# JohnsonLabJanelia/laserCalib

Hardware: NVIDIA B200
Metric: LM_iters_per_sec (higher is better)
Workload: dtype f64

## Files before the change

include/lcba.h:

```cpp
#ifndef LCBA_H
#define LCBA_H

#include <stddef.h>
#include <stdint.h>

#ifdef __cplusplus
extern "C" {
#endif

#define LCBA_VERSION 100
#define LCBA_CAM_PARAMS 11
#define LCBA_MAX_CAMERAS 64
#define LCBA_MAX_TRACE 512

enum {
  LCBA_OK = 0,
  LCBA_E_ARG = -1,
  LCBA_E_CUDA = -2,
  LCBA_E_STATE = -3,
  LCBA_E_UNSUPPORTED = -4,
  LCBA_E_NONFINITE = -5,
  LCBA_E_NCCL = -6
};

// ... 81 lines not shown

int lcba_residuals(lcba_t* h, const double* x_or_null, double* r_out, double* cost_out);

int lcba_jacobian_blocks(lcba_t* h, const double* x_or_null, double* Jc, double* Jp);

int lcba_sparsity_indices(lcba_t* h, int32_t C, int64_t P, int64_t N, const int64_t* cam_idx,
                          const int64_t* pt_idx, int32_t* indices_out);

int lcba_solve(lcba_t* h, const lcba_options* opt, lcba_result* res);
int lcba_get_trace(lcba_t* h, lcba_trace_row* rows, int32_t max_rows);
typedef void (*lcba_iteration_cb)(const lcba_trace_row* row, void* user);
int lcba_set_iteration_callback(lcba_t* h, lcba_iteration_cb cb, void* user);
int lcba_get_grad(lcba_t* h, double* g_out );
int lcba_get_profile(lcba_t* h, lcba_kernel_stat* stats, int32_t max_stats, int32_t* n_out);

int lcba_linearize(lcba_t* h, double lam, double* S_out, double* rhs_out, double* grad_out,
                   double* scale_inv_out, double* cost_out);

int lcba_time_device(lcba_t* h, int32_t what, int32_t reps, double* ms_out);

int lcba_nccl_unique_id(void* id_out128);
int lcba_comm_init(lcba_t* h, int32_t rank, int32_t nranks, const void* id128);

int lcba_debug_tr2d(double B00, double B01, double B11, double g0, double g1, double Delta,
                    double* p_out2, int* newton_out);

int lcba_debug_chol(lcba_t* h, int32_t n, const double* A, const double* rhs, double mu, const double* d,
                    int32_t grid, double* x_out, double* factor_out, int32_t* fail_out);

#define LCBA_STEP_SCALARS 18
int lcba_debug_step(lcba_t* h, double lam, double mu, int32_t mode, double* pc_out, double* pp_out,
                    double* scalars_out);

int lcba_debug_schur_stats(lcba_t* h, long long* out, int max_ctas, int* nkinds, int* nslices);

int lcba_debug_mma_plan(int32_t C, int32_t sm_count, int32_t* units_out, int32_t max_kinds,
                        int32_t* nslices_out, int32_t* ok_out);

int lcba_debug_i8_plan(int32_t C, int64_t P, int32_t sm_count, int32_t* tiles_out, int32_t max_tiles,
                       int32_t* work_out, int32_t max_work, int32_t* nwork_out, int32_t* nrg_out,
                       int64_t* nkb_out);

int lcba_debug_i8_cover_plan(int32_t C, int64_t P, int32_t sm_count, int32_t which, int32_t* tiles_out,
                             int32_t max_tiles, int32_t* work_out, int32_t max_work, int32_t* nwork_out,
                             int32_t* nrg_out, int64_t* nkb_out, int32_t* cover_out, double* model_out);

int lcba_debug_i8_fallback(lcba_t* h);

int lcba_debug_peer_reduce(lcba_t* h, int enable);

int lcba_host_is_nondecreasing_i64(const int64_t* v, int64_t n, int32_t threads);

#ifdef __cplusplus
}
#endif
#endif
```

lasercalib_b200/_cabi.py:

```python
from __future__ import annotations

import ctypes as C
import os

import numpy as np

_PKG = os.path.dirname(os.path.abspath(__file__))
LIB_PATH = os.path.join(_PKG, "liblcba.so")

LCBA_MAX_TRACE = 512
E_NAMES = {-1: "LCBA_E_ARG", -2: "LCBA_E_CUDA", -3: "LCBA_E_STATE", -4: "LCBA_E_UNSUPPORTED",
           -5: "LCBA_E_NONFINITE", -6: "LCBA_E_NCCL"}

SYMBOLS = ["lcba_version", "lcba_create", "lcba_destroy", "lcba_last_error", "lcba_default_options",
           "lcba_set_problem", "lcba_set_problem_shard", "lcba_set_params", "lcba_get_params", "lcba_rotate", "lcba_project",
           "lcba_unproject", "lcba_residuals", "lcba_jacobian_blocks", "lcba_sparsity_indices", "lcba_solve",
           "lcba_get_trace", "lcba_get_grad", "lcba_get_profile", "lcba_linearize",
           "lcba_time_device", "lcba_nccl_unique_id", "lcba_comm_init", "lcba_debug_tr2d",
           "lcba_sq_normal", "lcba_debug_schur_stats", "lcba_debug_mma_plan",
           "lcba_set_iteration_callback", "lcba_debug_i8_plan", "lcba_host_is_nondecreasing_i64", "lcba_debug_peer_reduce",
           "lcba_debug_i8_fallback", "lcba_debug_chol", "lcba_debug_step", "lcba_debug_i8_cover_plan"]

STEP_SCALARS = ["reg_term", "Delta", "Jg2", "aa", "ab", "bb", "JAA", "JAB", "JBB", "gtgt", "gtp", "pp",
                "c0", "c1", "predicted", "step_h_norm", "step_norm", "chol_fail"]


class Options(C.Structure):
    _fields_ = [("ftol", C.c_double), ("xtol", C.c_double), ("gtol", C.c_double),
                ("max_nfev", C.c_int64), ("verbose", C.c_int32), ("profile", C.c_int32),
                ("max_iterations", C.c_int32), ("fix_cameras", C.c_int32), ("shared_intrinsics", C.c_int32), ("reserved", C.c_int32 * 3)]


class TraceRow(C.Structure):
    _fields_ = [("iteration", C.c_int64), ("nfev", C.c_int64), ("cost", C.c_double),
                ("cost_reduction", C.c_double), ("step_norm", C.c_double),
                ("optimality", C.c_double), ("delta", C.c_double), ("reg_term", C.c_double)]


class Result(C.Structure):
    _fields_ = [("cost", C.c_double), ("optimality", C.c_double), ("initial_cost", C.c_double),
                ("nfev", C.c_int64), ("njev", C.c_int64), ("iterations", C.c_int64),
                ("status", C.c_int32), ("n_trace", C.c_int32), ("solve_ms", C.c_double),
                ("gpu_launches", C.c_int64), ("reserved", C.c_double * 6)]


class KernelStat(C.Structure):
    _fields_ = [("name", C.c_char * 32), ("launches", C.c_int64), ("total_ms", C.c_double)]


ITERATION_CB = C.CFUNCTYPE(None, C.POINTER(TraceRow), C.c_void_p)


def _row_dict(r):
    return dict(iteration=r.iteration, nfev=r.nfev, cost=r.cost, cost_reduction=r.cost_reduction,
# ... 29 lines not shown
    lib.lcba_default_options.argtypes = [C.POINTER(Options)]
    lib.lcba_default_options.restype = None
    lib.lcba_set_problem.argtypes = [vp, i32, i64, i64, vp, vp, vp, vp, vp, vp]
    lib.lcba_set_problem_shard.argtypes = [vp, i32, i64, i64, vp, vp, vp, vp, vp, vp, i64]
    lib.lcba_set_params.argtypes = [vp, vp, vp]
    lib.lcba_get_params.argtypes = [vp, vp, vp]
    lib.lcba_rotate.argtypes = [vp, i64, vp, vp, vp]
    lib.lcba_project.argtypes = [vp, i64, vp, vp, vp]
    lib.lcba_unproject.argtypes = [vp, i64, vp, vp, i64, vp, vp, vp, vp, vp]
    lib.lcba_residuals.argtypes = [vp, vp, vp, pd]
    lib.lcba_jacobian_blocks.argtypes = [vp, vp, vp, vp]
    lib.lcba_sparsity_indices.argtypes = [vp, i32, i64, i64, vp, vp, vp]
    lib.lcba_solve.argtypes = [vp, C.POINTER(Options), C.POINTER(Result)]
    lib.lcba_get_trace.argtypes = [vp, C.POINTER(TraceRow), i32]
    lib.lcba_set_iteration_callback.argtypes = [vp, ITERATION_CB, vp]
    lib.lcba_get_grad.argtypes = [vp, vp]
    lib.lcba_get_profile.argtypes = [vp, C.POINTER(KernelStat), i32, C.POINTER(i32)]
    lib.lcba_linearize.argtypes = [vp, dbl, vp, vp, vp, vp, pd]
    lib.lcba_time_device.argtypes = [vp, i32, i32, pd]
    lib.lcba_nccl_unique_id.argtypes = [vp]
    lib.lcba_comm_init.argtypes = [vp, i32, i32, vp]
    lib.lcba_sq_normal.argtypes = [vp, i32, vp, pd, vp, vp]
    lib.lcba_debug_mma_plan.argtypes = [i32, i32, vp, i32, C.POINTER(i32), C.POINTER(i32)]
    lib.lcba_debug_schur_stats.argtypes = [vp, vp, C.c_int, C.POINTER(C.c_int), C.POINTER(C.c_int)]
    lib.lcba_debug_i8_plan.argtypes = [i32, i64, i32, vp, i32, vp, i32, C.POINTER(i32), C.POINTER(i32), C.POINTER(i64)]
    lib.lcba_debug_i8_cover_plan.argtypes = [i32, i64, i32, i32, vp, i32, vp, i32, C.POINTER(i32), C.POINTER(i32),
                                             C.POINTER(i64), C.POINTER(i32), vp]
    lib.lcba_host_is_nondecreasing_i64.argtypes = [vp, i64, i32]
    lib.lcba_debug_peer_reduce.argtypes = [vp, i32]
    lib.lcba_debug_i8_fallback.argtypes = [vp]
    lib.lcba_debug_tr2d.argtypes = [dbl, dbl, dbl, dbl, dbl, dbl, pd, C.POINTER(C.c_int)]
    lib.lcba_debug_chol.argtypes = [vp, i32, vp, vp, dbl, vp, i32, vp, vp, C.POINTER(i32)]
    lib.lcba_debug_step.argtypes = [vp, dbl, dbl, i32, vp, vp, vp]
    _lib = lib
    return lib


def _ptr(a):
    return None if a is None else a.ctypes.data_as(C.c_void_p)


def _f64(a, shape=None):
    a = np.ascontiguousarray(a, dtype=np.float64)
    if shape is not None:
        a = a.reshape(shape)
    return a


def _i64(a):
    return np.ascontiguousarray(a, dtype=np.int64)


class Engine:

    def __init__(self, device=-1):
        self.lib = load()
        h = C.c_void_p()
        rc = self.lib.lcba_create(C.byref(h), int(device))
        if rc != 0:
            raise LcbaError(rc, self.lib.lcba_last_error(None).decode())
        self.h = h
        self.C = self.P = self.N = 0
        self.generation = 0

    def close(self):
        if getattr(self, "h", None):
            self.lib.lcba_destroy(self.h)
            self.h = None
# ... 176 lines not shown
                                          _ptr(work), work.shape[0], C.byref(nwork), C.byref(nrg), C.byref(nkb),
                                          C.byref(cover), _ptr(model))
        if nt < 0:
            raise LcbaError(nt, "lcba_debug_i8_cover_plan: bad arguments")
        return dict(tiles=tiles[:nt].copy(), work=work[:nwork.value].copy(), nrg=nrg.value, nkb=nkb.value,
                    cover=bool(cover.value), executed_ops=model[0], cycles=model[1], strip_cycles=model[2],
                    cover_cycles=model[3])

    def debug_chol(self, A, rhs, mu=0.0, d=None, grid=0):
        A = _f64(A)
        n = A.shape[0]
        if A.shape != (n, n):
            raise ValueError("A must be square")
        rhs = _f64(rhs).ravel()
        d = None if d is None else _f64(d).ravel()
        if rhs.size != n or (d is not None and d.size != n):
            raise ValueError("rhs and d must have n entries")
        x = np.empty(n)
        factor = np.empty((n + 1, n))
        fail = C.c_int32()
        self._check(self.lib.lcba_debug_chol(self.h, n, _ptr(A), _ptr(rhs), float(mu), _ptr(d), int(grid),
                                             _ptr(x), _ptr(factor), C.byref(fail)))
        return x, factor, fail.value

    STEP_FULL, STEP_FIX_CAMERAS, STEP_SHARED_INTRINSICS = 0, 1, 2

    def debug_step(self, lam, mu=0.0, mode=0):
        pc = np.empty(11 * self.C)
        pp = np.empty(3 * self.P)
        sc = np.empty(len(STEP_SCALARS))
        self._check(self.lib.lcba_debug_step(self.h, float(lam), float(mu), int(mode), _ptr(pc), _ptr(pp), _ptr(sc)))
        return pc, pp, dict(zip(STEP_SCALARS, sc.tolist()))

    def time_device(self, what, reps=10):
        ms = C.c_double()
        self._check(self.lib.lcba_time_device(self.h, int(what), int(reps), C.byref(ms)))
        return ms.value

    @staticmethod
    def nccl_unique_id():
        lib = load()
        buf = C.create_string_buffer(128)
        rc = lib.lcba_nccl_unique_id(buf)
        if rc != 0:
            raise LcbaError(rc, lib.lcba_last_error(None).decode())
        return buf.raw

    def comm_init(self, rank, nranks, unique_id=None):
        buf = None if unique_id is None else C.create_string_buffer(bytes(unique_id), 128)
        self._check(self.lib.lcba_comm_init(self.h, int(rank), int(nranks), buf))


def debug_tr2d(B00, B01, B11, g0, g1, Delta):
    lib = load()
    p = (C.c_double * 2)()
    newton = C.c_int()
    lib.lcba_debug_tr2d(B00, B01, B11, g0, g1, Delta, p, C.byref(newton))
    return np.array([p[0], p[1]]), bool(newton.value)
```

lasercalib_b200/csrc/lcba.cu:

```cuda
#include <dlfcn.h>
#include <math.h>
#include <stdio.h>
#include <string.h>
#include <algorithm>
#include <map>
#include <string>
#include <thread>
#include <vector>

#include <nvtx3/nvToolsExt.h>

#include "common.cuh"
#include "control.cuh"
#include "dense.cuh"
#include "eval.cuh"
#include "ingest.cuh"
#include "linearize.cuh"
#include "dense_passes.cuh"
#include "schur.cuh"
#include "schur_mma.cuh"
#include "schur_i8.cuh"
#include "peer_reduce.cuh"
#include "variants.cuh"

// ... 63 lines not shown
  double *d_S = nullptr, *d_Lf = nullptr, *d_rhs = nullptr, *d_Sred = nullptr, *d_Spart = nullptr;
  int* d_fail = nullptr;
  long long* d_stats = nullptr;
  Ctl* d_ctl = nullptr;
  Ctl* h_ctl = nullptr;
  int lin_grid = 0, obs_grid = 0, pt_grid = 0;
  SchurPlan plan;
  SchurKind* d_kinds = nullptr;
  SchurHw* d_hws = nullptr;
  MmaPlan mplan;
  MmaKind* d_mkinds = nullptr;
  double *d_U = nullptr, *d_Upart = nullptr;
  int camn_grid = 0, camn_pb = 0;
  bool use_mma = false;
  bool use_dense = false;
  bool use_pt = false;
  int pt_mode = 1;
  int ptp_grid = 0;
  int dp_pb = 0, dp_grid_lin = 0, dp_grid = 0;
  double *d_dpart = nullptr, *d_dred = nullptr;
  double* d_Yg = nullptr;
  bool use_i8 = false;
  bool i8_tma = false;
  I8Maps i8maps;
  I8Plan i8plan;
  I8Work* d_i8work = nullptr;
  I8Tile* d_i8tiles = nullptr;
  unsigned char* d_i8planes = nullptr;
  double *d_i8partial = nullptr, *d_i8rmax = nullptr;
  int* d_i8erow = nullptr;
  int* d_i8gate = nullptr;
  double* d_i8mrow = nullptr;
  bool i8_guard = true;
  int i8_gx_max = 0, i8_gx_make = 0, i8_groups = 0;
  double2* d_rout = nullptr;
  double *d_Jc = nullptr, *d_Jp = nullptr;
  uint32_t* d_pair_start = nullptr;
  double* d_pair_w = nullptr;
  long long n_pairs = 0;
  struct GraphSlot { cudaGraphExec_t exec = nullptr; long long launches = 0; int key = -1; };
  GraphSlot g_body[2], g_lin[2];
  bool use_graphs = true;
  int solves_on_problem = 0;
  long long graph_replays = 0;
  lcba_iteration_cb iter_cb = nullptr;
  void* iter_cb_user = nullptr;
  std::vector<lcba_trace_row> trace;
  bool prof_on = false;
  cudaEvent_t ev0 = nullptr, ev1 = nullptr;
  std::map<std::string, std::pair<long long, double>> prof;
  long long launches = 0;
  ncclComm_t comm = nullptr;
  int rank = 0, nranks = 1;
  int fix_cameras = 0, shared_intr = 0;
  double *d_pred = nullptr, *d_scl_red = nullptr;
  double *d_sqpart = nullptr, *d_sqout = nullptr, *d_theta = nullptr;
  int sq_grid = 0, sq_K = 0;
};

static std::string g_last_error;
static ncclComm_t g_comm = nullptr;
static int g_comm_rank = -1, g_comm_nranks = 0, g_comm_device = -1;
struct PeerState {
  bool ok = false;
  void* block = nullptr;
  void* opened[PEER_MAX_RANKS] = {};
  PeerPtrs ptrs = {};
// ... 122 lines not shown
    return LCBA_E_CUDA;
  }
  cudaDeviceProp prop;
  cudaGetDeviceProperties(&prop, device);
  h->sm_count = prop.multiProcessorCount;
  h->smem_optin = prop.sharedMemPerBlockOptin;
  cudaStreamCreateWithFlags(&h->stream, cudaStreamNonBlocking);
  {
    cudaMemPool_t pool;
    if (cudaDeviceGetDefaultMemPool(&pool, device) == cudaSuccess) {
      unsigned long long keep = ~0ull;
      cudaMemPoolSetAttribute(pool, cudaMemPoolAttrReleaseThreshold, &keep);
    }
  }
  cudaEventCreate(&h->ev0);
  cudaEventCreate(&h->ev1);
  cudaMallocHost((void**)&h->h_ctl, sizeof(Ctl));
  {
    const void* big_smem_kernels[] = {(const void*)k_linearize, (const void*)k_backsub,
                                      (const void*)k_schur<true, 160>, (const void*)k_schur<false, 160>,
                                      (const void*)k_schur<true, 128>, (const void*)k_schur<false, 128>,
                                      (const void*)k_residual, (const void*)k_cam_normal, (const void*)k_make_Y,
                                      (const void*)k_schur_mma<1, false>, (const void*)k_schur_mma<2, false>,
                                      (const void*)k_schur_mma<3, false>, (const void*)k_schur_mma<4, false>,
                                      (const void*)k_schur_mma<5, false>, (const void*)k_schur_mma<6, false>,
                                      (const void*)k_schur_mma<1, true>, (const void*)k_schur_mma<2, true>,
                                      (const void*)k_schur_mma<3, true>, (const void*)k_schur_mma<4, true>,
                                      (const void*)k_schur_mma<5, true>, (const void*)k_schur_mma<6, true>,
                                      (const void*)k_sq_camonly<true>, (const void*)k_sq_camonly<false>,
                                      (const void*)k_linearize_dense, (const void*)k_residual_dense,
                                      (const void*)k_jdot_dense, (const void*)k_backsub_dense,
                                      (const void*)k_residual_pt, (const void*)k_jdot_pt, (const void*)k_backsub_pt,
                                      (const void*)k_i8_syrk<true>, (const void*)k_i8_syrk<false>, (const void*)k_i8_make,
                                      (const void*)k_jdot,      (const void*)k_jacobian_blocks};
    for (const void* f : big_smem_kernels) {
      cudaFuncAttributes fa;
      e = cudaFuncGetAttributes(&fa, f);
      if (e == cudaSuccess)
        e = cudaFuncSetAttribute(f, cudaFuncAttributeMaxDynamicSharedMemorySize,
                                 (int)(h->smem_optin - fa.sharedSizeBytes));
      if (e != cudaSuccess) {
        set_error(nullptr, std::string("lcba_create: shared-memory opt-in: ") + cudaGetErrorString(e));
        delete h;
        return LCBA_E_CUDA;
      }
    }
  }
  *out = h;
  return LCBA_OK;
}

extern "C" void lcba_destroy(lcba_t* h) {
  if (!h) return;
  cudaSetDevice(h->device);
  h->comm = nullptr;
  dev_free_all(h);
  if (h->stream) cudaStreamSynchronize(h->stream);
  if (h->h_ctl) cudaFreeHost(h->h_ctl);
  if (h->ev0) cudaEventDestroy(h->ev0);
  if (h->ev1) cudaEventDestroy(h->ev1);
  if (h->stream) cudaStreamDestroy(h->stream);
  delete h;
}

static inline unsigned nblk(long long n, int t) { return (unsigned)std::max<long long>(1, (n + t - 1) / t); }

// ... 184 lines not shown
  LCBA_TRY(dev_alloc(h, &h->d_campart, (size_t)h->lin_grid * C * CAMSUM));
  LCBA_TRY(dev_alloc(h, &h->d_part, (size_t)max_grid * 16));
  h->plan = make_schur_plan(C, h->sm_count, h->smem_optin - 2048);
  LCBA_TRY(dev_alloc(h, &h->d_kinds, h->plan.kinds.size()));
  LCBA_TRY(dev_alloc(h, &h->d_hws, h->plan.hws.size()));
  LCBA_CUDA(h, cudaMemcpyAsync(h->d_kinds, h->plan.kinds.data(), h->plan.kinds.size() * sizeof(SchurKind),
                               cudaMemcpyHostToDevice, st));
  LCBA_CUDA(h, cudaMemcpyAsync(h->d_hws, h->plan.hws.data(), h->plan.hws.size() * sizeof(SchurHw),
                               cudaMemcpyHostToDevice, st));
  LCBA_TRY(dev_alloc(h, &h->d_Sred, h->plan.part_stride));
  h->use_mma = false;
  h->d_mkinds = nullptr; h->d_U = nullptr; h->d_Upart = nullptr; h->d_Yg = nullptr;
  int max_slices = h->plan.nslices;
  {
    const char* de = getenv("LCBA_MMA_DENSITY");
    const double min_density = de ? atof(de) : 0.25;
    const bool dense = (double)h->n_pairs >= min_density * (double)P * C;
    const char* env = getenv("LCBA_SCHUR_MMA");
    const bool want = env ? atoi(env) != 0 : (dense && C >= 8);
    if (want && C <= MMA_MAX_CAMERAS) {
      {
        const char* ie = getenv("LCBA_SCHUR_I8");
        h->use_i8 = ie ? atoi(ie) != 0 : P >= 32768;
      }
      if (h->use_i8) {
        {
          const char* pe = getenv("LCBA_I8_PLAN");
          const int which = !pe ? 0 : (strcmp(pe, "strip") == 0 ? 1 : (strcmp(pe, "cover") == 0 ? 2 : 0));
          h->i8plan = make_i8_best_plan(C, P, h->sm_count, which);
        }
        const I8Plan& ip = h->i8plan;
        h->i8_groups = (C + I8_GROUP_CAMS - 1) / I8_GROUP_CAMS;
        h->i8_gx_max = (int)std::max<long long>(1, std::min<long long>(ip.nkb, (long long)h->sm_count * 4 / h->i8_groups));
        h->i8_gx_make = (int)std::max<long long>(1, std::min<long long>(ip.nkb, (long long)h->sm_count * 3 / h->i8_groups));
        LCBA_TRY(dev_alloc(h, &h->d_i8work, ip.work.size()));
        LCBA_TRY(dev_alloc(h, &h->d_i8tiles, ip.tiles.size()));
        LCBA_CUDA(h, cudaMemcpyAsync(h->d_i8work, ip.work.data(), ip.work.size() * sizeof(I8Work), cudaMemcpyHostToDevice, st));
        LCBA_CUDA(h, cudaMemcpyAsync(h->d_i8tiles, ip.tiles.data(), ip.tiles.size() * sizeof(I8Tile), cudaMemcpyHostToDevice, st));
        LCBA_TRY(dev_alloc(h, &h->d_i8planes, ip.plane_bytes));
        {
          const char* te = getenv("LCBA_I8_TMA");
          h->i8_tma = !(te && atoi(te) == 0) && i8_encode_maps(ip, h->d_i8planes, &h->i8maps);
          if (!h->i8_tma) memset(&h->i8maps, 0, sizeof(h->i8maps));
        }
        LCBA_TRY(dev_alloc(h, &h->d_i8partial, ip.work.size() * 128 * 64));
        LCBA_TRY(dev_alloc(h, &h->d_i8rmax, (size_t)h->i8_gx_max * ip.NRG * 8));
        LCBA_TRY(dev_alloc(h, &h->d_i8erow, (size_t)ip.NRG * 8));
        LCBA_TRY(dev_alloc(h, &h->d_i8gate, 1));
        LCBA_TRY(dev_alloc(h, &h->d_i8mrow, (size_t)ip.NRG * 8));
        LCBA_CUDA(h, cudaMemsetAsync(h->d_i8gate, 0, sizeof(int), st));
        {
          const char* ge = getenv("LCBA_I8_GUARD");
          h->i8_guard = !(ge && atoi(ge) == 0);
        }
      }
      bool pre = false;
      if (!h->use_i8) {
        int rp = C * 12 + 2;
        while (rp % 16 != 4) ++rp;
        const size_t need = (size_t)(P + 1) * 3 * rp * 8;
        size_t fr = 0, tot = 0;
        const char* pe = getenv("LCBA_MMA_PRE");
        pre = cudaMemGetInfo(&fr, &tot) == cudaSuccess && need < fr / 3 && !(pe && atoi(pe) == 0);
        if (pre) LCBA_TRY(dev_alloc(h, &h->d_Yg, need / 8));
      }
      h->mplan = make_mma_plan(C, h->sm_count, h->smem_optin - 2048, !pre);
      LCBA_TRY(dev_alloc(h, &h->d_mkinds, h->mplan.kinds.size()));
// ... 273 lines not shown
        h->d_Vg, h->d_pts[w], h->d_scl_p, h->d_gt_p, h->P, first, h->d_part));
  KL(h, "reduce", k_reduce_scalars<<<PP_K, 256, 0, h->stream>>>(h->d_part, h->pt_grid, PP_K, pp, 3));
  LCBA_TRY(allreduce(h, h->d_camsum, (size_t)C * CAMSUM + 1 + 3, NCCL_SUM));
  LCBA_TRY(allreduce(h, pp + 3, 1, NCCL_MAX));
  KL(h, "ctl", k_ctl_lin<<<1, 256, 0, h->stream>>>(h->d_camsum, h->d_cams[w], h->d_scl_c, h->d_gt_c,
                                                   h->d_g_c, C, h->d_ctl, first, h->fix_cameras, h->shared_intr));
  KL(h, "ctl", k_ctl_lin2<<<1, 1, 0, h->stream>>>(pp, h->d_ctl, first));
  return check_launch(h, "linearize pass");
}

static int pass_jdot(lcba_t* h) {
  NvtxRange nvtx_("lcba:jdot");
  const int C = h->C, w = h->cur;
  const size_t smem = ((size_t)C * CAMTAB + (size_t)C * NCP) * 8;
  if (h->use_pt) {
    KL(h, "jdot", k_jdot_pt<<<h->ptp_grid, PT_THREADS, smem, h->stream>>>(
          h->d_tab[w], h->d_pts[w], h->d_w, h->d_obs_start, h->d_mask, h->d_gt_c, h->d_gt_p, h->P, C, h->d_part));
    KL(h, "reduce", k_reduce_scalars<<<1, 256, 0, h->stream>>>(h->d_part, h->ptp_grid, 1, h->d_red, 1));
  } else if (h->use_dense && h->pt_mode == 2) {
    KL(h, "jdot", k_jdot_dense<<<h->dp_grid, DP_THREADS, (size_t)C * CAMTAB * 8, h->stream>>>(
          h->d_tab[w], h->d_pts[w], h->d_w, h->d_obs_start, h->d_mask, h->d_gt_c, h->d_gt_p, h->P, C,
          h->dp_pb, h->d_part));
    KL(h, "reduce", k_reduce_scalars<<<1, 256, 0, h->stream>>>(h->d_part, h->dp_grid, 1, h->d_red, 1));
  } else {
  KL(h, "jdot", k_jdot<<<h->obs_grid, 256, smem, h->stream>>>(
        h->d_tab[w], h->d_pts[w], h->d_cam, h->d_pt, h->d_w, h->d_gt_c, h->d_gt_p, h->N, C, h->d_part));
  KL(h, "reduce", k_reduce_scalars<<<1, 256, 0, h->stream>>>(h->d_part, h->obs_grid, 1, h->d_red, 1));
  }
  LCBA_TRY(allreduce(h, h->d_red, 1, NCCL_SUM));
  KL(h, "ctl", k_ctl_reg<<<1, 1, 0, h->stream>>>(h->d_red, h->d_ctl));
  return check_launch(h, "jdot pass");
}

static int pass_schur(lcba_t* h, const double* lam_host_or_null) {
  NvtxRange nvtx_("lcba:schur");
  const int C = h->C, w = h->cur, n = C * NCP;
  const SchurPlan& pl = h->plan;
  const double lam_arg = lam_host_or_null ? *lam_host_or_null : 0.0;
  const Ctl* ctl_arg = lam_host_or_null ? nullptr : h->d_ctl;
  KL(h, "point_factor", k_point_factor<<<nblk(h->P, 256), 256, 0, h->stream>>>(
        h->d_Vg, h->d_scl_p, lam_arg, ctl_arg, h->P, h->d_Lz));
  if (h->use_mma) {
    const MmaPlan& mp = h->mplan;
    if (!h->use_dense) {
    const size_t smem_u = ((size_t)((C * CAMTAB + 1) & ~1) + (size_t)h->camn_pb * C) * 8;
    KL(h, "cam_normal", k_cam_normal<<<h->camn_grid, 256, smem_u, h->stream>>>(
          h->d_tab[w], h->d_pts[w], h->d_pair_w, h->d_pair_start, h->d_mask, h->P, C, h->camn_pb, h->d_Upart));
    KL(h, "reduce", k_reduce_cols<<<nblk(C * CAMN_VALS, RC_COLS), RC_COLS * RC_ROWS, 0, h->stream>>>(
          h->d_Upart, h->camn_grid, C * CAMN_VALS, h->d_U));
    }
    const int nt = (NCP * C + 1 + 7) / 8, last = nt - 6 * ((nt + 5) / 6 - 1);
    if (h->use_i8) {
      const I8Plan& ip = h->i8plan;
      const int RP = ip.NRG * 8;
      const size_t smem_rm = ((size_t)I8_GROUP_CAMS * CAMTAB + 192) * 4;
      KL(h, "i8_rowmax", k_i8_rowmax<<<dim3(h->i8_gx_max, h->i8_groups), 192, smem_rm, h->stream>>>(
            h->d_tab[w], h->d_pts[w], h->d_pair_w, h->d_pair_start, h->d_mask, h->d_Lz, h->P, C, RP, h->d_i8rmax));
      KL(h, "i8_rowmax", k_i8_rowexp<<<nblk(RP, 128), 128, 0, h->stream>>>(h->d_i8rmax, h->i8_gx_max, NCP * C + 1, RP,
                                                                     h->d_i8erow, h->d_i8mrow));
      KL(h, "make_Y", k_i8_make<<<dim3(h->i8_gx_make, h->i8_groups), 192, i8_make_smem_bytes(), h->stream>>>(
            h->d_tab[w], h->d_pts[w], h->d_pair_w, h->d_pair_start, h->d_mask, h->d_Lz, h->P, C, ip.NRG, h->d_i8erow,
            h->d_i8planes));
      if (h->i8_tma)
        KL(h, "schur", k_i8_syrk<true><<<(unsigned)ip.work.size(), I8_THREADS, ip.smem_bytes, h->stream>>>(
              h->i8maps, h->d_i8planes, ip.NRG, h->d_i8work, h->d_i8partial, h->d_fail, h->d_stats));
      else
        KL(h, "schur", k_i8_syrk<false><<<(unsigned)ip.work.size(), I8_THREADS, ip.smem_bytes, h->stream>>>(
              h->i8maps, h->d_i8planes, ip.NRG, h->d_i8work, h->d_i8partial, h->d_fail, h->d_stats));
      KL(h, "schur_reduce", k_i8_gather<<<dim3((unsigned)ip.tiles.size(), 16), 256, 0, h->stream>>>(
            h->d_i8partial, h->d_i8tiles, C, ip.cover ? 1 : 0, h->d_i8erow, pl.npairs, h->d_Sred));
      KL(h, "schur_reduce", k_add_cam_blocks<<<nblk(C * 121, 128), 128, 0, h->stream>>>(h->d_U, C, h->d_Sred));
      if (h->i8_guard) {
        KL(h, "i8_check", k_i8_check<<<1, 256, 0, h->stream>>>(h->d_i8mrow, C, h->d_Sred, h->d_i8gate));
#define LCBA_MMA_GATED(L)                                                                            \
  KL(h, "i8_fallback", (k_schur_mma<L, false><<<dim3(mp.nslices, mp.nkinds), MMA_THREADS, mp.smem_bytes, h->stream>>>( \
          nullptr, h->d_tab[w], h->d_pts[w], h->d_pair_w, h->d_pair_start, h->d_mask, h->d_Lz, h->P, h->n_pairs, C, \
          h->d_mkinds, mp.nslices, pl.part_stride, pl.npairs, h->d_Spart, nullptr, h->d_i8gate)))
        switch (last) {
          case 1: LCBA_MMA_GATED(1); break;
          case 2: LCBA_MMA_GATED(2); break;
          case 3: LCBA_MMA_GATED(3); break;
          case 4: LCBA_MMA_GATED(4); break;
          case 5: LCBA_MMA_GATED(5); break;
          default: LCBA_MMA_GATED(6); break;
        }
#undef LCBA_MMA_GATED
        KL(h, "i8_fallback", k_i8_fallback_finish<<<h->sm_count, 256, 0, h->stream>>>(
              h->d_i8gate, h->d_Spart, mp.nslices, pl.part_stride, h->d_U, C, h->d_Sred));
      }
    } else {
    if (h->d_Yg) {
      const int pbk = MAKEY_THREADS / C, rpk = mp.kinds[0].rp;
      const size_t smem_y = ((size_t)((C * CAMTAB + 1) & ~1) + (size_t)3 * pbk * rpk) * 8;
      const int grid_y = (int)std::min<long long>((h->P + pbk - 1) / pbk, (long long)h->sm_count * 5);
      KL(h, "make_Y", k_make_Y<<<grid_y, MAKEY_THREADS, smem_y, h->stream>>>(
// ... 832 lines not shown
  if (mode < 0 || mode > 2) { set_error(h, "lcba_debug_step: mode must be 0, 1 or 2"); return LCBA_E_ARG; }
  cudaSetDevice(h->device);
  Ctl init;
  memset(&init, 0, sizeof(init));
  init.term = -1;
  LCBA_CUDA(h, cudaMemcpyAsync(h->d_ctl, &init, sizeof(Ctl), cudaMemcpyHostToDevice, h->stream));
  h->fix_cameras = mode == 1 ? 1 : 0;
  h->shared_intr = mode == 2 ? 1 : 0;
  LCBA_TRY(pass_linearize(h, 1));
  LCBA_TRY(pass_jdot(h));
  if (h->fix_cameras) {
    KL(h, "point_factor", k_point_factor<<<nblk(h->P, 256), 256, 0, h->stream>>>(
          h->d_Vg, h->d_scl_p, lam, nullptr, h->P, h->d_Lz));
    LCBA_CUDA(h, cudaMemsetAsync(h->d_pc, 0, (size_t)h->C * NCP * 8, h->stream));
    LCBA_CUDA(h, cudaMemsetAsync(h->d_fail, 0, 2 * sizeof(int), h->stream));
  } else {
    LCBA_TRY(pass_schur(h, &lam));
    LCBA_TRY(pass_camera_solve(h, mu));
  }
  LCBA_TRY(pass_backsub(h));
  if (pc_out) LCBA_CUDA(h, cudaMemcpyAsync(pc_out, h->d_pc, (size_t)h->C * NCP * 8, cudaMemcpyDeviceToHost, h->stream));
  if (pp_out) LCBA_CUDA(h, cudaMemcpyAsync(pp_out, h->d_gn_p, (size_t)h->P * 3 * 8, cudaMemcpyDeviceToHost, h->stream));
  LCBA_TRY(read_ctl(h));
  if (scalars_out) {
    const Ctl& c = *h->h_ctl;
    const double v[LCBA_STEP_SCALARS] = {c.reg_term, c.Delta, c.Jg2, c.aa, c.ab, c.bb, c.JAA, c.JAB, c.JBB,
                                         c.gtgt, c.gtp, c.pp, c.c0, c.c1, c.predicted, c.step_h_norm,
                                         c.step_norm, (double)c.chol_fail};
    memcpy(scalars_out, v, sizeof(v));
  }
  return LCBA_OK;
}

extern "C" int lcba_host_is_nondecreasing_i64(const int64_t* v, int64_t n, int32_t threads) {
  if (!v || n < 2) return 1;
  const int nt = (int)std::max<int64_t>(1, std::min<int64_t>(std::min<int64_t>(threads, 16), n / (1 << 20)));
  std::vector<int> ok(nt, 1);
  auto piece = [&](int i) {
    const int64_t a = n * i / nt, b = std::min<int64_t>(n, n * (i + 1) / nt + 1);
    int64_t bad = 0;
    for (int64_t k = a + 1; k < b; ++k) bad |= (int64_t)(v[k] < v[k - 1]);
    ok[i] = bad ? 0 : 1;
  };
  if (nt == 1) { piece(0); return ok[0]; }
  std::vector<std::thread> th;
  int started = 1;
  try {
    for (int i = 1; i < nt; ++i) { th.emplace_back(piece, i); started = i + 1; }
  } catch (...) {
  }
  piece(0);
  for (int i = started; i < nt; ++i) piece(i);
  for (auto& t : th) t.join();
  for (int i = 0; i < nt; ++i) if (!ok[i]) return 0;
  return 1;
}
```

lasercalib_b200/csrc/schur_i8.cuh:

```cuda
#pragma once
#include <cuda.h>
#include <algorithm>
#include <vector>
#include "common.cuh"
#include "schur_mma.cuh"

namespace lcba {

constexpr int I8_NS = 6;
constexpr int I8_DMAX = 6;
constexpr int I8_ND = I8_DMAX + 1;
constexpr int I8_PTS = 21;
constexpr int I8_STAGES = 3;
constexpr int I8_FLUSH = 224;
constexpr int I8_THREADS = 192;
constexpr int I8_RG_BYTES = 512;
constexpr int I8_GROUP_CAMS = 8;
constexpr int I8_GROUP_RG = 13;
constexpr int I8_GROUP_ROWS = I8_GROUP_RG * 8;

struct I8Work {
  int m_rg0, m_nrg, m2_rg0, m2_nrg, n_rg0, n_nrg, n2_rg0, n2_nrg;
  int kb0, kb1;
  int map_a, map_b1, map_b2, pad;
// ... 363 lines not shown
      for (int qq = 0; qq < I8_PTS; ++qq) m = fmaxf(m, s_red[qq * gc + t]);
      out[(c0 + t) * NCP + a] = (double)m;
    }
  }
  if (g == gridDim.y - 1) {
    __syncthreads();
    s_red[t] = zthread ? mz : 0.0f;
    __syncthreads();
    if (t == 0) {
      float m = 0.0f;
      for (int i = 168; i < 168 + I8_PTS; ++i) m = fmaxf(m, s_red[i]);
      out[NCP * C] = (double)m;
    }
  }
}

__global__ void k_i8_rowexp(const double* __restrict__ rmax_part, int nb, int R, int RP, int* __restrict__ e_row,
                            double* __restrict__ m_row) {
  const int r = blockIdx.x * blockDim.x + threadIdx.x;
  if (r >= RP) return;
  double m = 0.0;
  if (r < R) for (int b = 0; b < nb; ++b) m = fmax(m, rmax_part[(size_t)b * RP + r]);
  int e = 0;
  if (m > 0.0 && m < 1e300) { frexp(m * 1.001, &e); e += 2; }
  e_row[r] = e;
  m_row[r] = m;
}

__device__ __forceinline__ unsigned long long i8_encode(double v, double scale) {
  const long long T = __double2ll_rn(v * scale);
  return (unsigned long long)(T + 0x808080808080LL) ^ 0x808080808080ULL;
}

constexpr int I8_VAL_LD = 65;
inline size_t i8_make_smem_bytes() {
  return (size_t)I8_GROUP_CAMS * CAMTAB * 8 + (size_t)I8_GROUP_ROWS * 8 + (size_t)I8_GROUP_ROWS * I8_VAL_LD * 8;
}

__global__ void __launch_bounds__(192, 3)
k_i8_make(const double* __restrict__ tab, const double* __restrict__ pts, const double* __restrict__ wgt,
          const uint32_t* __restrict__ obs_start, const unsigned long long* __restrict__ mask,
          const double* __restrict__ Lz, long long P, int C, int NRG, const int* __restrict__ e_row,
          unsigned char* __restrict__ planes) {
  extern __shared__ __align__(16) unsigned char s_raw[];
  double* s_tab = reinterpret_cast<double*>(s_raw);
  double* s_scale = s_tab + I8_GROUP_CAMS * CAMTAB;
  unsigned long long* s_val = reinterpret_cast<unsigned long long*>(s_scale + I8_GROUP_ROWS);
  const int t = threadIdx.x, g = blockIdx.y, lane = t & 31, wid = t >> 5;
  const int c0 = g * I8_GROUP_CAMS, gc = min(I8_GROUP_CAMS, C - c0);
  const int rg0 = 11 * g;
  const int nrgl = (g == (int)gridDim.y - 1) ? NRG - rg0 : 11;
  for (int i = t; i < gc * CAMTAB; i += blockDim.x) s_tab[i] = tab[c0 * CAMTAB + i];
  for (int i = t; i < I8_GROUP_ROWS; i += blockDim.x)
    s_scale[i] = (rg0 * 8 + i < NRG * 8) ? ldexp(1.0, 8 * I8_NS - e_row[rg0 * 8 + i]) : 0.0;
  for (int i = t; i < I8_GROUP_ROWS * I8_VAL_LD; i += blockDim.x) s_val[i] = 0ull;
  __syncthreads();
  const bool worker = t < I8_PTS * gc;
  const int slot = worker ? t / gc : 0;
  const int q = slot < 16 ? (slot >> 1) + 8 * (slot & 1) : slot, cl = worker ? t % gc : 0, cam = c0 + cl;
  const bool zthread = (g == (int)gridDim.y - 1) && t >= 168 && t < 168 + I8_PTS;
  const int zrow = NCP * C - rg0 * 8;
  const long long nkb = (P + I8_PTS - 1) / I8_PTS;
  unsigned long long n_m = 0ull;
  double n_X[3] = {0, 0, 0}, n_li[6] = {0, 0, 0, 0, 0, 0};
  auto prefetch = [&](long long kb) {
    n_m = 0ull;
    const long long p = kb * I8_PTS + q;
    if (worker && kb < nkb && p < P) {
      n_m = mask[p];
#pragma unroll
      for (int a = 0; a < 3; ++a) n_X[a] = pts[3 * p + a];
#pragma unroll
      for (int a = 0; a < 6; ++a) n_li[a] = Lz[p * 9 + a];
// ... 43 lines not shown
      for (int k = 0; k < 3; ++k)
        s_val[(size_t)zrow * I8_VAL_LD + 3 * qq + k] = p < P ? i8_encode(Lz[p * 9 + 6 + k], s_scale[zrow]) : 0ull;
    }
    __syncthreads();
    {
      const int kh = lane >> 4, r8 = (lane >> 1) & 7, hf = lane & 1;
      const size_t sstride = (size_t)NRG * I8_RG_BYTES;
      unsigned char* lane_dst = planes + (((size_t)kb * I8_NS) * NRG + rg0) * I8_RG_BYTES + kh * 128 + r8 * 16 + hf * 8;
      const unsigned long long* lane_src = s_val + (size_t)r8 * I8_VAL_LD + kh * 16 + hf * 8;
      for (int task = wid; task < nrgl * 2; task += 6) {
        const int rgl = task >> 1, a = task & 1;
        const unsigned long long* src = lane_src + (size_t)rgl * 8 * I8_VAL_LD + a * 32;
        unsigned lo[8], hi[8];
#pragma unroll
        for (int e = 0; e < 8; ++e) { const unsigned long long v = src[e]; lo[e] = (unsigned)v; hi[e] = (unsigned)(v >> 32); }
        unsigned char* dst = lane_dst + (size_t)rgl * I8_RG_BYTES + a * 256;
#pragma unroll
        for (int i = 0; i < I8_NS; ++i) {
          const unsigned sel = i == 0 ? 0x0051u : i == 1 ? 0x0040u : i == 2 ? 0x0073u : i == 3 ? 0x0062u : i == 4 ? 0x0051u : 0x0040u;
          unsigned w[2];
#pragma unroll
          for (int h2 = 0; h2 < 2; ++h2) {
            const unsigned* x = (i < 2) ? hi + 4 * h2 : lo + 4 * h2;
            w[h2] = __byte_perm(__byte_perm(x[0], x[1], sel), __byte_perm(x[2], x[3], sel), 0x5410);
          }
          *reinterpret_cast<uint2*>(dst + (size_t)i * sstride) = make_uint2(w[0], w[1]);
        }
      }
    }
    __syncthreads();
  }
}

struct I8Op { int i, j, nj, fresh, coll; };
template <int NCOL, bool FIRST>
struct I8KstepPlan {
  I8Op ops[32];
  int n;
  constexpr I8KstepPlan() : ops{}, n(0) {
    bool touched[I8_ND] = {};
    for (int i = I8_NS - 1; i >= 0; --i) {
      if (i > I8_DMAX) continue;
      const int jmax = (I8_NS - 1 < I8_DMAX - i) ? I8_NS - 1 : I8_DMAX - i;
      if (FIRST) {
        for (int j = 0; j <= jmax; ++j) {
          ops[n].i = i; ops[n].j = j; ops[n].nj = 1; ops[n].fresh = touched[i + j] ? 0 : 1; ops[n].coll = 0;
          touched[i + j] = true;
          ++n;
        }
      } else {
        const int per = 256 / NCOL, cnt = jmax + 1;
        int j = 0, rem = cnt % per;
        while (j <= jmax) {
          const int nj = (rem > 0) ? rem : per;
          rem = 0;
          ops[n].i = i; ops[n].j = j; ops[n].nj = nj; ops[n].fresh = 0; ops[n].coll = 0;
          ++n;
          j += nj;
        }
      }
    }
    for (int q = 0; q < n; ++q) {
      const bool prev = q > 0 && ops[q - 1].i == ops[q].i, next = q + 1 < n && ops[q + 1].i == ops[q].i;
      ops[q].coll = prev ? (next ? 2 : 3) : (next ? 1 : 0);
    }
  }
// ... 264 lines not shown
```

Before: 136.7.

## Warp-specialize i8 plane builder with double-buffered smem producer/consumer pipeline

```diff
diff --git a/include/lcba.h b/include/lcba.h
--- a/include/lcba.h
+++ b/include/lcba.h
@@ -137,6 +137,9 @@
 int lcba_debug_step(lcba_t* h, double lam, double mu, int32_t mode, double* pc_out, double* pp_out,
                     double* scalars_out);
 
+int lcba_debug_i8_make(lcba_t* h, double lam, int32_t ref, int32_t reps, int32_t poison, double* ms_out,
+                       void* planes_out, int64_t planes_bytes);
+
 int lcba_debug_schur_stats(lcba_t* h, long long* out, int max_ctas, int* nkinds, int* nslices);
 
 int lcba_debug_mma_plan(int32_t C, int32_t sm_count, int32_t* units_out, int32_t max_kinds,
diff --git a/lasercalib_b200/_cabi.py b/lasercalib_b200/_cabi.py
--- a/lasercalib_b200/_cabi.py
+++ b/lasercalib_b200/_cabi.py
@@ -19,7 +19,8 @@
            "lcba_time_device", "lcba_nccl_unique_id", "lcba_comm_init", "lcba_debug_tr2d",
            "lcba_sq_normal", "lcba_debug_schur_stats", "lcba_debug_mma_plan",
            "lcba_set_iteration_callback", "lcba_debug_i8_plan", "lcba_host_is_nondecreasing_i64", "lcba_debug_peer_reduce",
-           "lcba_debug_i8_fallback", "lcba_debug_chol", "lcba_debug_step", "lcba_debug_i8_cover_plan"]
+           "lcba_debug_i8_fallback", "lcba_debug_chol", "lcba_debug_step", "lcba_debug_i8_cover_plan",
+           "lcba_debug_i8_make"]
 
 STEP_SCALARS = ["reg_term", "Delta", "Jg2", "aa", "ab", "bb", "JAA", "JAB", "JBB", "gtgt", "gtp", "pp",
                 "c0", "c1", "predicted", "step_h_norm", "step_norm", "chol_fail"]
@@ -115,8 +116,15 @@
     lib.lcba_debug_tr2d.argtypes = [dbl, dbl, dbl, dbl, dbl, dbl, pd, C.POINTER(C.c_int)]
     lib.lcba_debug_chol.argtypes = [vp, i32, vp, vp, dbl, vp, i32, vp, vp, C.POINTER(i32)]
     lib.lcba_debug_step.argtypes = [vp, dbl, dbl, i32, vp, vp, vp]
+    lib.lcba_debug_i8_make.argtypes = [vp, dbl, i32, i32, i32, pd, vp, i64]
     _lib = lib
     return lib
+
+
+def i8_plane_bytes(n_cams, n_points):
+    nrg = (11 * n_cams + 1 + 7) // 8
+    nrg += nrg & 1
+    return -(-n_points // 21) * 6 * nrg * 512
 
 
 def _ptr(a):
@@ -359,6 +367,16 @@
         self._check(self.lib.lcba_debug_step(self.h, float(lam), float(mu), int(mode), _ptr(pc), _ptr(pp), _ptr(sc)))
         return pc, pp, dict(zip(STEP_SCALARS, sc.tolist()))
 
+    def debug_i8_make(self, lam, ref=False, reps=1, planes=True, poison=0xA5):
+        ms = C.c_double()
+        buf, nbytes = None, 0
+        if planes:
+            nbytes = i8_plane_bytes(self.C, self.P)
+            buf = np.empty(nbytes, dtype=np.uint8)
+        self._check(self.lib.lcba_debug_i8_make(self.h, float(lam), int(bool(ref)), int(reps),
+                                                -1 if poison is None else int(poison), C.byref(ms), _ptr(buf), nbytes))
+        return ms.value, buf
+
     def time_device(self, what, reps=10):
         ms = C.c_double()
         self._check(self.lib.lcba_time_device(self.h, int(what), int(reps), C.byref(ms)))
diff --git a/lasercalib_b200/csrc/lcba.cu b/lasercalib_b200/csrc/lcba.cu
--- a/lasercalib_b200/csrc/lcba.cu
+++ b/lasercalib_b200/csrc/lcba.cu
@@ -119,7 +119,7 @@
   int* d_i8gate = nullptr;
   double* d_i8mrow = nullptr;
   bool i8_guard = true;
-  int i8_gx_max = 0, i8_gx_make = 0, i8_groups = 0;
+  int i8_gx_max = 0, i8_gx_make = 0, i8_gx_make_ref = 0, i8_groups = 0;
   double2* d_rout = nullptr;
   double *d_Jc = nullptr, *d_Jp = nullptr;
   uint32_t* d_pair_start = nullptr;
@@ -308,6 +308,7 @@
                                       (const void*)k_jdot_dense, (const void*)k_backsub_dense,
                                       (const void*)k_residual_pt, (const void*)k_jdot_pt, (const void*)k_backsub_pt,
                                       (const void*)k_i8_syrk<true>, (const void*)k_i8_syrk<false>, (const void*)k_i8_make,
+                                      (const void*)k_i8_make_ref,
                                       (const void*)k_jdot,      (const void*)k_jacobian_blocks};
     for (const void* f : big_smem_kernels) {
       cudaFuncAttributes fa;
@@ -558,7 +559,8 @@
         const I8Plan& ip = h->i8plan;
         h->i8_groups = (C + I8_GROUP_CAMS - 1) / I8_GROUP_CAMS;
         h->i8_gx_max = (int)std::max<long long>(1, std::min<long long>(ip.nkb, (long long)h->sm_count * 4 / h->i8_groups));
-        h->i8_gx_make = (int)std::max<long long>(1, std::min<long long>(ip.nkb, (long long)h->sm_count * 3 / h->i8_groups));
+        h->i8_gx_make = (int)std::max<long long>(1, std::min<long long>(ip.nkb, (long long)h->sm_count * 2 / h->i8_groups));
+        h->i8_gx_make_ref = (int)std::max<long long>(1, std::min<long long>(ip.nkb, (long long)h->sm_count * 3 / h->i8_groups));
         LCBA_TRY(dev_alloc(h, &h->d_i8work, ip.work.size()));
         LCBA_TRY(dev_alloc(h, &h->d_i8tiles, ip.tiles.size()));
         LCBA_CUDA(h, cudaMemcpyAsync(h->d_i8work, ip.work.data(), ip.work.size() * sizeof(I8Work), cudaMemcpyHostToDevice, st));
@@ -898,6 +900,26 @@
   return check_launch(h, "jdot pass");
 }
 
+static void launch_i8_rowexp(lcba_t* h) {
+  const int C = h->C, w = h->cur, RP = h->i8plan.NRG * 8;
+  const size_t smem_rm = ((size_t)I8_GROUP_CAMS * CAMTAB + 192) * 4;
+  KL(h, "i8_rowmax", k_i8_rowmax<<<dim3(h->i8_gx_max, h->i8_groups), 192, smem_rm, h->stream>>>(
+        h->d_tab[w], h->d_pts[w], h->d_pair_w, h->d_pair_start, h->d_mask, h->d_Lz, h->P, C, RP, h->d_i8rmax));
+  KL(h, "i8_rowmax", k_i8_rowexp<<<nblk(RP, 128), 128, 0, h->stream>>>(h->d_i8rmax, h->i8_gx_max, NCP * C + 1, RP,
+                                                                 h->d_i8erow, h->d_i8mrow));
+}
+static void launch_i8_make(lcba_t* h, bool ref) {
+  const int C = h->C, w = h->cur, NRG = h->i8plan.NRG;
+  if (ref)
+    KL(h, "make_Y", k_i8_make_ref<<<dim3(h->i8_gx_make_ref, h->i8_groups), 192, i8_make_ref_smem_bytes(), h->stream>>>(
+          h->d_tab[w], h->d_pts[w], h->d_pair_w, h->d_pair_start, h->d_mask, h->d_Lz, h->P, C, NRG, h->d_i8erow,
+          h->d_i8planes));
+  else
+    KL(h, "make_Y", k_i8_make<<<dim3(h->i8_gx_make, h->i8_groups), I8_MK_THREADS, i8_make_smem_bytes(), h->stream>>>(
+          h->d_tab[w], h->d_pts[w], h->d_pair_w, h->d_pair_start, h->d_mask, h->d_Lz, h->P, C, NRG, h->d_i8erow,
+          h->d_i8planes));
+}
+
 static int pass_schur(lcba_t* h, const double* lam_host_or_null) {
   NvtxRange nvtx_("lcba:schur");
   const int C = h->C, w = h->cur, n = C * NCP;
@@ -918,15 +940,8 @@
     const int nt = (NCP * C + 1 + 7) / 8, last = nt - 6 * ((nt + 5) / 6 - 1);
     if (h->use_i8) {
       const I8Plan& ip = h->i8plan;
-      const int RP = ip.NRG * 8;
-      const size_t smem_rm = ((size_t)I8_GROUP_CAMS * CAMTAB + 192) * 4;
-      KL(h, "i8_rowmax", k_i8_rowmax<<<dim3(h->i8_gx_max, h->i8_groups), 192, smem_rm, h->stream>>>(
-            h->d_tab[w], h->d_pts[w], h->d_pair_w, h->d_pair_start, h->d_mask, h->d_Lz, h->P, C, RP, h->d_i8rmax));
-      KL(h, "i8_rowmax", k_i8_rowexp<<<nblk(RP, 128), 128, 0, h->stream>>>(h->d_i8rmax, h->i8_gx_max, NCP * C + 1, RP,
-                                                                     h->d_i8erow, h->d_i8mrow));
-      KL(h, "make_Y", k_i8_make<<<dim3(h->i8_gx_make, h->i8_groups), 192, i8_make_smem_bytes(), h->stream>>>(
-            h->d_tab[w], h->d_pts[w], h->d_pair_w, h->d_pair_start, h->d_mask, h->d_Lz, h->P, C, ip.NRG, h->d_i8erow,
-            h->d_i8planes));
+      launch_i8_rowexp(h);
+      launch_i8_make(h, false);
       if (h->i8_tma)
         KL(h, "schur", k_i8_syrk<true><<<(unsigned)ip.work.size(), I8_THREADS, ip.smem_bytes, h->stream>>>(
               h->i8maps, h->d_i8planes, ip.NRG, h->d_i8work, h->d_i8partial, h->d_fail, h->d_stats));
@@ -1825,6 +1840,45 @@
   return LCBA_OK;
 }
 
+extern "C" int lcba_debug_i8_make(lcba_t* h, double lam, int32_t ref, int32_t reps, int32_t poison, double* ms_out,
+                                  void* planes_out, int64_t planes_bytes) {
+  if (!h || !h->have_problem) { set_error(h, "lcba_debug_i8_make: no problem set"); return LCBA_E_STATE; }
+  if (!h->use_i8) { set_error(h, "lcba_debug_i8_make: the problem does not take the int8 path (LCBA_SCHUR_I8)"); return LCBA_E_STATE; }
+  if (ref < 0 || ref > 1 || reps < 1 || poison < -1 || poison > 255 ||
+      (planes_out && planes_bytes != (int64_t)h->i8plan.plane_bytes)) {
+    set_error(h, "lcba_debug_i8_make: ref must be 0 or 1, reps >= 1, poison -1..255, planes_bytes = " +
+                     std::to_string(h->i8plan.plane_bytes));
+    return LCBA_E_ARG;
+  }
+  cudaSetDevice(h->device);
+  Ctl init;
+  memset(&init, 0, sizeof(init));
+  init.term = -1;
+  LCBA_CUDA(h, cudaMemcpyAsync(h->d_ctl, &init, sizeof(Ctl), cudaMemcpyHostToDevice, h->stream));
+  LCBA_TRY(pass_linearize(h, 1));
+  KL(h, "point_factor", k_point_factor<<<nblk(h->P, 256), 256, 0, h->stream>>>(
+        h->d_Vg, h->d_scl_p, lam, nullptr, h->P, h->d_Lz));
+  launch_i8_rowexp(h);
+  if (poison >= 0) LCBA_CUDA(h, cudaMemsetAsync(h->d_i8planes, poison, h->i8plan.plane_bytes, h->stream));
+  cudaEvent_t e0, e1;
+  LCBA_CUDA(h, cudaEventCreate(&e0));
+  if (cudaEventCreate(&e1) != cudaSuccess) { cudaEventDestroy(e0); set_error(h, "lcba_debug_i8_make: cudaEventCreate"); return LCBA_E_CUDA; }
+  cudaError_t e = cudaEventRecord(e0, h->stream);
+  for (int r = 0; r < reps && e == cudaSuccess; ++r) launch_i8_make(h, ref != 0);
+  if (e == cudaSuccess) e = cudaGetLastError();
+  if (e == cudaSuccess) e = cudaEventRecord(e1, h->stream);
+  if (e == cudaSuccess && planes_out)
+    e = cudaMemcpyAsync(planes_out, h->d_i8planes, h->i8plan.plane_bytes, cudaMemcpyDeviceToHost, h->stream);
+  if (e == cudaSuccess) e = cudaStreamSynchronize(h->stream);
+  float ms = 0.0f;
+  if (e == cudaSuccess) e = cudaEventElapsedTime(&ms, e0, e1);
+  cudaEventDestroy(e0);
+  cudaEventDestroy(e1);
+  if (e != cudaSuccess) { set_error(h, std::string("lcba_debug_i8_make: ") + cudaGetErrorString(e)); return LCBA_E_CUDA; }
+  if (ms_out) *ms_out = (double)ms / reps;
+  return LCBA_OK;
+}
+
 extern "C" int lcba_host_is_nondecreasing_i64(const int64_t* v, int64_t n, int32_t threads) {
   if (!v || n < 2) return 1;
   const int nt = (int)std::max<int64_t>(1, std::min<int64_t>(std::min<int64_t>(threads, 16), n / (1 << 20)));
diff --git a/lasercalib_b200/csrc/schur_i8.cuh b/lasercalib_b200/csrc/schur_i8.cuh
--- a/lasercalib_b200/csrc/schur_i8.cuh
+++ b/lasercalib_b200/csrc/schur_i8.cuh
@@ -419,13 +419,18 @@
   return (unsigned long long)(T + 0x808080808080LL) ^ 0x808080808080ULL;
 }
 
+__device__ __forceinline__ unsigned long long i8_encode_fma(double v, double scale) {
+  const unsigned long long T = (unsigned long long)__double_as_longlong(fma(v, scale, 6755399441055744.0));
+  return (T + 0x808080808080ULL) ^ 0x808080808080ULL;
+}
+
 constexpr int I8_VAL_LD = 65;
-inline size_t i8_make_smem_bytes() {
+inline size_t i8_make_ref_smem_bytes() {
   return (size_t)I8_GROUP_CAMS * CAMTAB * 8 + (size_t)I8_GROUP_ROWS * 8 + (size_t)I8_GROUP_ROWS * I8_VAL_LD * 8;
 }
 
 __global__ void __launch_bounds__(192, 3)
-k_i8_make(const double* __restrict__ tab, const double* __restrict__ pts, const double* __restrict__ wgt,
+k_i8_make_ref(const double* __restrict__ tab, const double* __restrict__ pts, const double* __restrict__ wgt,
           const uint32_t* __restrict__ obs_start, const unsigned long long* __restrict__ mask,
           const double* __restrict__ Lz, long long P, int C, int NRG, const int* __restrict__ e_row,
           unsigned char* __restrict__ planes) {
@@ -535,6 +540,175 @@
   }
 }
 
+constexpr int I8_MK_EVAL = 192;
+constexpr int I8_MK_DRAIN = 64;
+constexpr int I8_MK_THREADS = I8_MK_EVAL + I8_MK_DRAIN;
+constexpr int I8_MK_LDL = 68;
+constexpr int I8_MK_LDH = 72;
+constexpr int I8_MK_LO = I8_GROUP_ROWS * I8_MK_LDL;
+constexpr int I8_MK_HI = I8_GROUP_ROWS * I8_MK_LDH;
+inline size_t i8_make_smem_bytes() {
+  return (size_t)I8_GROUP_CAMS * CAMTAB * 8 + (size_t)I8_GROUP_ROWS * 8 + 2 * ((size_t)I8_MK_LO * 4 + (size_t)I8_MK_HI * 2);
+}
+template <int ID> __device__ __forceinline__ void i8_bar_sync() { asm volatile("bar.sync %0, %1;" ::"n"(ID), "n"(I8_MK_THREADS) : "memory"); }
+template <int ID> __device__ __forceinline__ void i8_bar_arrive() { asm volatile("bar.arrive %0, %1;" ::"n"(ID), "n"(I8_MK_THREADS) : "memory"); }
+
+__global__ void __launch_bounds__(I8_MK_THREADS, 2)
+k_i8_make(const double* __restrict__ tab, const double* __restrict__ pts, const double* __restrict__ wgt,
+          const uint32_t* __restrict__ obs_start, const unsigned long long* __restrict__ mask,
+          const double* __restrict__ Lz, long long P, int C, int NRG, const int* __restrict__ e_row,
+          unsigned char* __restrict__ planes) {
+  extern __shared__ __align__(16) unsigned char s_raw[];
+  double* s_tab = reinterpret_cast<double*>(s_raw);
+  double* s_scale = s_tab + I8_GROUP_CAMS * CAMTAB;
+  uint32_t* s_lo = reinterpret_cast<uint32_t*>(s_scale + I8_GROUP_ROWS);
+  uint16_t* s_hi = reinterpret_cast<uint16_t*>(s_lo + 2 * I8_MK_LO);
+  constexpr int BAR_FULL = 1, BAR_EMPTY = 3;
+  const int t = threadIdx.x, g = blockIdx.y;
+  const int c0 = g * I8_GROUP_CAMS, gc = min(I8_GROUP_CAMS, C - c0);
+  const int rg0 = 11 * g;
+  const int nrgl = (g == (int)gridDim.y - 1) ? NRG - rg0 : 11;
+  for (int i = t; i < gc * CAMTAB; i += blockDim.x) s_tab[i] = tab[c0 * CAMTAB + i];
+  for (int i = t; i < I8_GROUP_ROWS; i += blockDim.x)
+    s_scale[i] = (rg0 * 8 + i < NRG * 8) ? ldexp(1.0, 8 * I8_NS - e_row[rg0 * 8 + i]) : 0.0;
+  {
+    uint4* z = reinterpret_cast<uint4*>(s_lo);
+    const int n16 = (2 * I8_MK_LO * 4 + 2 * I8_MK_HI * 2) / 16;
+    for (int i = t; i < n16; i += blockDim.x) z[i] = make_uint4(0u, 0u, 0u, 0u);
+  }
+  __syncthreads();
+  const long long nkb = (P + I8_PTS - 1) / I8_PTS;
+  const long long G = gridDim.x;
+
+  if (t < I8_MK_EVAL) {
+    const bool worker = t < I8_PTS * gc;
+    const int q = worker ? t / gc : 0, cl = worker ? t % gc : 0, cam = c0 + cl;
+    const bool zthread = (g == (int)gridDim.y - 1) && t >= 168 && t < 168 + I8_PTS;
+    const int zrow = NCP * C - rg0 * 8;
+    const unsigned long long below = (1ull << cam) - 1ull;
+    unsigned long long a_m = 0ull;
+    uint32_t a_os = 0u;
+    auto prefetch2 = [&](long long kb) {
+      a_m = 0ull;
+      const long long p = kb * I8_PTS + q;
+      if (worker && kb < nkb && p < P) { a_m = mask[p]; a_os = wgt ? obs_start[p] : 0u; }
+    };
+    unsigned long long n_m = 0ull;
+    double n_X[3] = {0, 0, 0}, n_li[6] = {0, 0, 0, 0, 0, 0}, n_w = 1.0;
+    auto prefetch1 = [&](long long kb) {
+      n_m = a_m;
+      const long long p = kb * I8_PTS + q;
+      if (worker && kb < nkb && p < P) {
+#pragma unroll
+        for (int a = 0; a < 3; ++a) n_X[a] = pts[3 * p + a];
+#pragma unroll
+        for (int a = 0; a < 6; ++a) n_li[a] = Lz[p * 9 + a];
+        if (wgt && ((n_m >> cam) & 1ull)) n_w = wgt[(long long)a_os + __popcll(n_m & below)];
+      }
+    };
+    prefetch2(blockIdx.x);
+    prefetch1(blockIdx.x);
+    prefetch2(blockIdx.x + G);
+    int it = 0;
+    for (long long kb = blockIdx.x; kb < nkb; kb += G, ++it) {
+      const int b = it & 1;
+      const unsigned long long m = n_m;
+      const bool live = (m >> cam) & 1ull;
+      const double w = n_w;
+      double X[3], li[6];
+#pragma unroll
+      for (int a = 0; a < 3; ++a) X[a] = n_X[a];
+#pragma unroll
+      for (int a = 0; a < 6; ++a) li[a] = n_li[a];
+      prefetch1(kb + G);
+      prefetch2(kb + 2 * G);
+      if (it >= 2) { if (b) i8_bar_sync<BAR_EMPTY + 1>(); else i8_bar_sync<BAR_EMPTY>(); }
+      uint32_t* lo = s_lo + b * I8_MK_LO;
+      uint16_t* hi = s_hi + b * I8_MK_HI;
+      if (worker) {
+        uint32_t* dlo = lo + (cl * NCP) * I8_MK_LDL + 3 * q;
+        uint16_t* dhi = hi + (cl * NCP) * I8_MK_LDH + 3 * q;
+        if (live) {
+          ObsLin L;
+          obs_linearize<false>(s_tab + cl * CAMTAB, X[0], X[1], X[2], 0.0, 0.0, w, L);
+          const double* sc = s_scale + cl * NCP;
+#pragma unroll
+          for (int k = 0; k < 3; ++k) {
+            double q0, q1;
+            if (k == 0) { q0 = L.Jp[0][0] * li[0]; q1 = L.Jp[1][0] * li[0]; }
+            else if (k == 1) { q0 = fma(L.Jp[0][0], li[1], L.Jp[0][1] * li[2]); q1 = fma(L.Jp[1][0], li[1], L.Jp[1][1] * li[2]); }
+            else { q0 = fma(L.Jp[0][0], li[3], fma(L.Jp[0][1], li[4], L.Jp[0][2] * li[5]));
+                   q1 = fma(L.Jp[1][0], li[3], fma(L.Jp[1][1], li[4], L.Jp[1][2] * li[5])); }
+#pragma unroll
+            for (int a = 0; a < NCP; ++a) {
+              const double y = a < 9 ? fma(L.Jc[0][a], q0, L.Jc[1][a] * q1) : (a == 9 ? w * q0 : w * q1);
+              const unsigned long long v = i8_encode_fma(y, sc[a]);
+              dlo[a * I8_MK_LDL + k] = (uint32_t)v;
+              dhi[a * I8_MK_LDH + k] = (uint16_t)(v >> 32);
+            }
+          }
+        } else {
+#pragma unroll
+          for (int k = 0; k < 3; ++k)
+#pragma unroll
+            for (int a = 0; a < NCP; ++a) { dlo[a * I8_MK_LDL + k] = 0u; dhi[a * I8_MK_LDH + k] = 0u; }
+        }
+      }
+      if (zthread) {
+        const int qq = t - 168;
+        const long long pz = kb * I8_PTS + qq;
+#pragma unroll
+        for (int k = 0; k < 3; ++k) {
+          const unsigned long long v = pz < P ? i8_encode_fma(Lz[pz * 9 + 6 + k], s_scale[zrow]) : 0ull;
+          lo[zrow * I8_MK_LDL + 3 * qq + k] = (uint32_t)v;
+          hi[zrow * I8_MK_LDH + 3 * qq + k] = (uint16_t)(v >> 32);
+        }
+      }
+      __threadfence_block();
+      if (b) i8_bar_arrive<BAR_FULL + 1>(); else i8_bar_arrive<BAR_FULL>();
+    }
+  } else {
+    const int lane = t & 31, dw = (t - I8_MK_EVAL) >> 5;
+    const int r8 = lane & 7, kh = (lane >> 3) & 1, a = lane >> 4;
+    const int kap = 32 * a + 16 * kh;
+    const size_t sstride = (size_t)NRG * I8_RG_BYTES;
+    int it = 0;
+    for (long long kb = blockIdx.x; kb < nkb; kb += G, ++it) {
+      const int b = it & 1;
+      if (b) i8_bar_sync<BAR_FULL + 1>(); else i8_bar_sync<BAR_FULL>();
+      const uint32_t* lo = s_lo + b * I8_MK_LO + r8 * I8_MK_LDL + kap;
+      const uint16_t* hi = s_hi + b * I8_MK_HI + r8 * I8_MK_LDH + kap;
+      unsigned char* lane_dst = planes + (((size_t)kb * I8_NS) * NRG + rg0) * I8_RG_BYTES + a * 256 + kh * 128 + r8 * 16;
+      for (int rgl = dw; rgl < nrgl; rgl += I8_MK_DRAIN / 32) {
+        const uint4* sl = reinterpret_cast<const uint4*>(lo + rgl * 8 * I8_MK_LDL);
+        const uint4* sh = reinterpret_cast<const uint4*>(hi + rgl * 8 * I8_MK_LDH);
+        uint32_t x[16], hw[8];
+#pragma unroll
+        for (int j = 0; j < 4; ++j) { const uint4 u = sl[j]; x[4 * j] = u.x; x[4 * j + 1] = u.y; x[4 * j + 2] = u.z; x[4 * j + 3] = u.w; }
+#pragma unroll
+        for (int j = 0; j < 2; ++j) { const uint4 u = sh[j]; hw[4 * j] = u.x; hw[4 * j + 1] = u.y; hw[4 * j + 2] = u.z; hw[4 * j + 3] = u.w; }
+        uint32_t out[I8_NS][4];
+#pragma unroll
+        for (int j = 0; j < 4; ++j) {
+          out[0][j] = __byte_perm(hw[2 * j], hw[2 * j + 1], 0x7531);
+          out[1][j] = __byte_perm(hw[2 * j], hw[2 * j + 1], 0x6420);
+          const uint32_t t0 = __byte_perm(x[4 * j], x[4 * j + 1], 0x5140), t1 = __byte_perm(x[4 * j + 2], x[4 * j + 3], 0x5140);
+          const uint32_t t2 = __byte_perm(x[4 * j], x[4 * j + 1], 0x7362), t3 = __byte_perm(x[4 * j + 2], x[4 * j + 3], 0x7362);
+          out[2][j] = __byte_perm(t2, t3, 0x7632);
+          out[3][j] = __byte_perm(t2, t3, 0x5410);
+          out[4][j] = __byte_perm(t0, t1, 0x7632);
+          out[5][j] = __byte_perm(t0, t1, 0x5410);
+        }
+        unsigned char* dst = lane_dst + (size_t)rgl * I8_RG_BYTES;
+#pragma unroll
+        for (int i = 0; i < I8_NS; ++i)
+          *reinterpret_cast<uint4*>(dst + (size_t)i * sstride) = make_uint4(out[i][0], out[i][1], out[i][2], out[i][3]);
+      }
+      if (kb + 2 * G < nkb) { if (b) i8_bar_arrive<BAR_EMPTY + 1>(); else i8_bar_arrive<BAR_EMPTY>(); }
+    }
+  }
+}
+
 struct I8Op { int i, j, nj, fresh, coll; };
 template <int NCOL, bool FIRST>
 struct I8KstepPlan {
```

New measurement: 140.9 (median of 6 runs). +3.0%, better.
